# OthmanB/TAMCMC-C-

Measured on AMD Instinct MI355X. Metric: MALA steps/sec (all chains) + achieved HBM GB/s, 64 chains × 1e5-bin spectrum, higher is better.
Workload: dtype f64; 1 GPU; C2: model_MS_Global_a1etaa3_HarveyLike (id 2), 21 modes l=0..2, 56 params, 100000 bins, 64 chains per GPU, trunc_c=20, logL + gradient over 44 variables, params resident in HBM; chains_total=64

## Files before the change

### tamcmc-c-_amd/csrc/tamcmc_dev.h

```cpp
#pragma once
#include <stddef.h>
#include <stdint.h>
#if defined(__HIPCC__)
#define TM_HD __host__ __device__
#else
#define TM_HD
#endif

#define TM_MAXM 7
#define TM_MAXH 3
#define TM_THREADS 256
#define TM_MAXMULT 256
#define TM_GSLOTS 24
#define TM_NSLOTS 16
#define TM_PDEG 8
#define TM_ORDER_MAX 1024
#define TM_HSER 10

#define TM_FAM_GAUSS  0
#define TM_FAM_GLOBAL 1
#define TM_FAM_LOCAL  2

struct TmLayout {
    int32_t model_case;
    int32_t family;
    int32_t variant;
    int32_t Nmax, lmax;
    int32_t Nfl[4];
    int32_t Nsplit, Nwidth, Nnoise, Ninc;
    int32_t off_f[4];
    int32_t s, w, z, q;
    int32_t Nparams;
    int32_t n_mult;
    int32_t nharvey;
    int32_t likelihood_case;
    int32_t Nx;
    int32_t bg_exact;
    int32_t asym_var;
    int32_t pad_l;
    double  x0, xlast, step;
    double  like_p;
};

struct TmMult {
    double g2;
    double aA, aB, c2;
    double nu2[TM_MAXM];
    double hq[TM_MAXM];
    int32_t imin, imax;
    int32_t ncomp;
    int32_t has_asym;
};
static_assert(sizeof(TmMult) == 160, "TmMult layout");
#define TM_MULT_DOUBLES 20

struct TmNoise {
    double H[TM_MAXH];
    double lt[TM_MAXH];
    double p[TM_MAXH];
    double N0;
    double gA, gnu0, gs2;
    int32_t nh;
    int32_t has_gauss;
    int32_t status;
    int32_t pad;
};

static_assert(sizeof(TmNoise) == 120, "TmNoise layout");
#define TM_NOISE_DOUBLES 15

#define TM_UNIT_BINS 512
#define TM_UNIT_SHIFT 9
#define TM_CELL_UNITS 8
#define TM_CELL_SHIFT 3
#ifndef TM_TILE_MAXU
#define TM_TILE_MAXU 8
#endif
#define TM_TILE_MAXU_L 16
#define TM_EQ_MAXU 4096

struct TmCellRec {
    double bg[TM_PDEG + 1];
    double t0[TM_MAXH];
    double lxc;
    int32_t npoly;
    int32_t pad;
};
static_assert(sizeof(TmCellRec) == 8 * (TM_PDEG + 1 + TM_MAXH + 2), "TmCellRec layout");

struct TmTileHdr {
    int32_t u0, u1, nact, cost;
};
static_assert(sizeof(TmTileHdr) == 16, "TmTileHdr layout");

struct TmActive {
    int32_t idx;
    int32_t imin, imax;
    int32_t shape;
};
static_assert(sizeof(TmActive) == 16, "TmActive layout");

struct TmCostModel {
    int32_t c0, a, b, pad;
    int32_t t1, su1, su2, pad2;
};
static inline TM_HD int tm_tile_first_unit(const TmCostModel &g, int su, int t) { return (g.t1 <= 0) ? t * su : (t < g.t1 ? t * g.su1 : g.t1 * g.su1 + (t - g.t1) * g.su2); }
static inline TM_HD int tm_tile_units(const TmCostModel &g, int su, int t) { return (g.t1 <= 0) ? su : (t < g.t1 ? g.su1 : g.su2); }
static inline TM_HD int tm_tile_of_unit(const TmCostModel &g, int su, int u) { return (g.t1 <= 0) ? u / su : (u < g.t1 * g.su1 ? u / g.su1 : g.t1 + (u - g.t1 * g.su1) / g.su2); }

struct TmEvalArgs {
    const double *x2, *y, *lx, *isig2;
    const TmMult *mult;
    const TmNoise *noise;
    const TmCellRec *cell;
    const TmTileHdr *thdr;
    const TmActive *tidx;
    const int32_t *spec;
    const double *wt;
    double *part;
    double *gmult;
    double *gnoise;
    int32_t *ticket;
    double *logL;
    int32_t *status;
    const int32_t *row_of_chain;
    double *model_out;
    int32_t Nx, n_mult, tiles, cells, likelihood_case;
    const int32_t *order;
    int32_t order_mode;
    int32_t prio;
    int32_t generic;
    double like_p;
    unsigned long long tile_magic;
};

static inline int tm_units(long long Nx) { return (int)((Nx + TM_UNIT_BINS - 1) / TM_UNIT_BINS); }
static inline int tm_cells(int units) { return (units + TM_CELL_UNITS - 1) / TM_CELL_UNITS; }
static inline int tm_tiles(int units, int grad)
{
    (void)grad;
    if (units <= 4) return 1;
    if (units < 70) { const int s = units / 10 > 0 ? units / 10 : 1; return (units + s - 1) / s; }
    return (units + TM_TILE_MAXU - 1) / TM_TILE_MAXU;
}

#if defined(__HIPCC__)
#define TM_LN2 0.693147180559945309417232
static __device__ __forceinline__ double tm_tile_logsum(double mant, double e) { return __builtin_fma(e, TM_LN2, log(mant)); }
#endif
static inline TM_HD int tm_setup_balances(int units, int tiles, int equal_cost, int max_units_per_tile)
{
    return (equal_cost != 0 && max_units_per_tile == TM_TILE_MAXU && tiles > 1 && tiles <= TM_ORDER_MAX && units <= TM_EQ_MAXU &&
            (long long)tiles * TM_TILE_MAXU > units) ? 1 : 0;
}

static inline TM_HD int tm_tile_bound(int t, int tiles, int units, const int *pre, long long C, long long cmin)
{
    const long long T = tiles, U = units, S = TM_TILE_MAXU;
    const long long D = T * S - U;
    const long long Nl = (C - T * S * cmin > 0) ? C - T * S * cmin : 0;
    const long long rhs = (long long)t * (D * C + Nl * U);
    int lo = 0, hi = units;
    while (lo < hi) {
        const int mid = (lo + hi) >> 1;
        const long long q = (mid == 0) ? 0 : (long long)pre[mid - 1];
        if (T * (D * q + Nl * mid) >= rhs) hi = mid; else lo = mid + 1;
    }
    return lo;
}

struct TmFusedArgs {
    const double *params, *Tcoefs;
    void *chain_rec, *aux;
    double *hser;
    int32_t p_doubles, pad;
};

#ifdef __cplusplus
extern "C++" {
struct ihipStream_t;
int tm_launch_setup(const TmLayout &L, int Nchains, const double *d_params, const double *d_Tcoefs, double *d_wt, const double *d_lx,
                    int units, int cells, int tiles, int equal_cost, TmCostModel cm, TmMult *d_mult, TmNoise *d_noise, TmCellRec *d_cell,
                    TmTileHdr *d_thdr, TmActive *d_tidx, void *d_chain_rec , void *d_aux ,
                    double *d_hser , int32_t *d_order , void *stream);
size_t tm_sizeof_chain_rec();
size_t tm_sizeof_aux();
int tm_launch_eval(const TmEvalArgs &a, int Nchains, bool grad, void *stream);
int tm_launch_fused(const TmLayout &L, const TmFusedArgs &f, const TmEvalArgs &a, int Nchains, bool grad, void *stream);
int tm_launch_backward(const TmLayout &L, int Nchains, int units, int cells, int tiles, int equal_cost ,
                       TmCostModel geom ,
                       const double *d_params,
                       const double *d_Tcoefs, const void *d_chain_rec, const void *d_aux, const TmNoise *d_noise,
                       const double *d_part, const double *d_gmult, const double *d_gnoise, const TmCellRec *d_cell,
                       const TmTileHdr *d_thdr, const double *d_hser, int Nvars, const int32_t *d_index_to_relax, double *d_grad,
                       double *d_logL, int32_t *d_status, void *stream);
int tm_backward_fits(const TmLayout &L, int tiles, int Nvars);
}
#endif
```

### tamcmc-c-_amd/csrc/tamcmc_eval_body.h

```cpp
#ifndef TAMCMC_EVAL_BODY_H
#define TAMCMC_EVAL_BODY_H
#include <hip/hip_runtime.h>
#include "tamcmc_dev.h"

#define TM_WAVES (TM_THREADS / 64)

typedef const __attribute__((address_space(4))) TmMult *TmMultK;
typedef const __attribute__((address_space(4))) TmCellRec *TmCellRecK;
typedef const __attribute__((address_space(4))) TmTileHdr *TmTileHdrK;
typedef const __attribute__((address_space(4))) TmNoise *TmNoiseK;
typedef const __attribute__((address_space(4))) int32_t *TmIdxK;
typedef const __attribute__((address_space(4))) TmActive *TmActiveK;

typedef int TmEntry __attribute__((ext_vector_type(4)));
__device__ __forceinline__ TmEntry tm_load_entry(TmActiveK p)
{
    return *reinterpret_cast<const __attribute__((address_space(4))) TmEntry *>(p);
}

__device__ __forceinline__ double tm_rcp(double x)
{
    double r = __builtin_amdgcn_rcp(x);
    double e = __builtin_fma(-x, r, 1.0);
    r = __builtin_fma(r, e, r);
    e = __builtin_fma(-x, r, 1.0);
    r = __builtin_fma(r, e, r);
    return r;
}

__device__ __forceinline__ double tm_rcp1(double x)
{
    double r = __builtin_amdgcn_rcp(x);
    const double e = __builtin_fma(-x, r, 1.0);
    return __builtin_fma(r, e, r);
}

template <int MASK>
__device__ __forceinline__ unsigned tm_xor_dw(unsigned v, int lane)
{
    if constexpr (MASK == 1) return __builtin_amdgcn_update_dpp(0u, v, 0xB1, 0xf, 0xf, false);
    else if constexpr (MASK == 2) return __builtin_amdgcn_update_dpp(0u, v, 0x4E, 0xf, 0xf, false);
    else if constexpr (MASK == 4) {
        const unsigned r = __builtin_amdgcn_update_dpp(0u, v, 0x104, 0xf, 0x5, false);
        return __builtin_amdgcn_update_dpp(r, v, 0x114, 0xf, 0xa, false);
    } else if constexpr (MASK == 8) return __builtin_amdgcn_update_dpp(0u, v, 0x128, 0xf, 0xf, false);
    else if constexpr (MASK == 16) {
        const auto r = __builtin_amdgcn_permlane16_swap(v, v, false, false);
        return (lane & 16) ? r[0] : r[1];
    } else {
        const auto r = __builtin_amdgcn_permlane32_swap(v, v, false, false);
        return (lane & 32) ? r[0] : r[1];
    }
}

template <int MASK>
__device__ __forceinline__ double tm_xor(double v, int lane)
{
    const unsigned long long b = __double_as_longlong(v);
    const unsigned lo = tm_xor_dw<MASK>((unsigned)b, lane), hi = tm_xor_dw<MASK>((unsigned)(b >> 32), lane);
    return __longlong_as_double(((unsigned long long)hi << 32) | lo);
}

template <int MASK>
__device__ __forceinline__ double tm_swap_add(double a, double b)
{
    static_assert(MASK == 16 || MASK == 32, "two-register swaps exist for 16 and 32 lanes");
    const unsigned long long ba = __double_as_longlong(a), bb = __double_as_longlong(b);
    unsigned r0l, r1l, r0h, r1h;
    if constexpr (MASK == 32) {
        const auto l = __builtin_amdgcn_permlane32_swap((unsigned)ba, (unsigned)bb, false, false);
        const auto h = __builtin_amdgcn_permlane32_swap((unsigned)(ba >> 32), (unsigned)(bb >> 32), false, false);
        r0l = l[0]; r1l = l[1]; r0h = h[0]; r1h = h[1];
    } else {
        const auto l = __builtin_amdgcn_permlane16_swap((unsigned)ba, (unsigned)bb, false, false);
        const auto h = __builtin_amdgcn_permlane16_swap((unsigned)(ba >> 32), (unsigned)(bb >> 32), false, false);
        r0l = l[0]; r1l = l[1]; r0h = h[0]; r1h = h[1];
    }
    const double r0 = __longlong_as_double(((unsigned long long)r0h << 32) | r0l);
    const double r1 = __longlong_as_double(((unsigned long long)r1h << 32) | r1l);
    return r0 + r1;
}

__device__ __forceinline__ double tm_wave_sum(double v)
{
    const int lane = threadIdx.x & 63;
    v += tm_xor<32>(v, lane);
    v += tm_xor<16>(v, lane);
    v += tm_xor<8>(v, lane);
    v += tm_xor<4>(v, lane);
    v += tm_xor<2>(v, lane);
    v += tm_xor<1>(v, lane);
    return v;
}

__device__ __forceinline__ double tm_wave_prod(double v)
{
    const int lane = threadIdx.x & 63;
    v *= tm_xor<32>(v, lane);
    v *= tm_xor<16>(v, lane);
    v *= tm_xor<8>(v, lane);
    v *= tm_xor<4>(v, lane);
    v *= tm_xor<2>(v, lane);
    v *= tm_xor<1>(v, lane);
    return v;
}


__device__ __forceinline__ double tm_poly(TmCellRecK tr, double z)
{
    double p = tr->bg[TM_PDEG];
#pragma unroll
    for (int j = TM_PDEG - 1; j >= 0; j--) p = __builtin_fma(p, z, tr->bg[j]);
    return p;
}

template <int N, int MASK>
struct TmBfly {
    static constexpr int NE = (N + 1) & ~1;
    static constexpr int H = NE / 2;
    __device__ static __forceinline__ void run(double (&v)[TM_GSLOTS], int lane)
    {
        if constexpr (N == 1) {
            v[0] += tm_xor<MASK>(v[0], lane);
        } else if constexpr (MASK >= 16) {
#pragma unroll
            for (int i = 0; i < H; i++) v[i] = tm_swap_add<MASK>(v[i], (i + H < N) ? v[i + H] : 0.0);
        } else {
            const bool hi = (lane & MASK) != 0;
#pragma unroll
            for (int i = 0; i < H; i++) {
                const double up = (i + H < N) ? v[i + H] : 0.0;
                const double send = hi ? v[i] : up;
                const double keep = hi ? up : v[i];
                v[i] = keep + tm_xor<MASK>(send, lane);
            }
        }
        if constexpr (MASK > 1) TmBfly<(N == 1 ? 1 : H), MASK / 2>::run(v, lane);
    }
    __device__ static __forceinline__ int slot_of(int lane, bool &valid)
    {
        if constexpr (N == 1) {
            return 0;
        } else {
            int sub = 0;
            if constexpr (MASK > 1) sub = TmBfly<H, MASK / 2>::slot_of(lane, valid);
            const int idx = sub + (((lane & MASK) != 0) ? H : 0);
            if (idx >= N) valid = false;
            return idx;
        }
    }
};

template <int NC>
__device__ __forceinline__ double tm_mult_value(double x2, const double (&nu2)[NC], const double (&hq)[NC], double g2,
                                                double (&d)[NC], double (&r)[NC])
{
    double E[NC], P[NC];
#pragma unroll
    for (int m = 0; m < NC; m++) {
        d[m] = x2 - nu2[m];
        E[m] = __builtin_fma(d[m], d[m], g2);
    }
    P[0] = E[0];
#pragma unroll
    for (int m = 1; m < NC; m++) P[m] = P[m - 1] * E[m];
    double inv = tm_rcp1(P[NC - 1]);
    double s = 0.0;
#pragma unroll
    for (int m = NC - 1; m >= 1; m--) {
        r[m] = inv * P[m - 1];
        inv = inv * E[m];
    }
    r[0] = inv;
#pragma unroll
    for (int m = 0; m < NC; m++) s = __builtin_fma(hq[m], r[m], s);
    return s;
}

template <int NC>
__device__ __forceinline__ double tm_mult_sum(double x2, const double (&nu2)[NC], const double (&hq)[NC], double g2)
{
    double d = x2 - nu2[0];
    double Q = __builtin_fma(d, d, g2);
    double N = hq[0];
#pragma unroll
    for (int m = 1; m < NC; m++) {
        d = x2 - nu2[m];
        const double E = __builtin_fma(d, d, g2);
        N = __builtin_fma(hq[m], Q, N * E);
        Q = Q * E;
    }
    return N * tm_rcp(Q);
}

template <int NC, int KG, bool ASYM>
__device__ __forceinline__ void tm_accum_mult(TmMultK sm, const double (&x2)[KG], const int (&bi)[KG], double (&acc)[KG], const bool edge)
{
    double nu2[NC], hq[NC];
#pragma unroll
    for (int m = 0; m < NC; m++) { nu2[m] = sm->nu2[m]; hq[m] = sm->hq[m]; }
    const double g2 = sm->g2;
    const double aAh = ASYM ? 0.5 * sm->aA : 0.0, aB = ASYM ? sm->aB : 1.0, c2 = ASYM ? sm->c2 : 0.0;
    double s[KG];
#pragma unroll
    for (int k = 0; k < KG; k++) {
        s[k] = tm_mult_sum<NC>(x2[k], nu2, hq, g2);
        if (ASYM) {
            const double a = __builtin_fma(x2[k], aAh, aB);
            s[k] = s[k] * __builtin_fma(a, a, c2);
        }
    }
    if (edge) {
        const int imin = sm->imin, imax = sm->imax;
#pragma unroll
        for (int k = 0; k < KG; k++) {
            const bool inside = (bi[k] >= imin) && (bi[k] < imax);
            s[k] = inside ? s[k] : 0.0;
        }
    }
#pragma unroll
    for (int k = 0; k < KG; k++) acc[k] += s[k];
}

template <int KG>
__device__ __forceinline__ void tm_accum_dispatch(TmMultK sm, const int shape, const double (&x2)[KG], const int (&bi)[KG], double (&acc)[KG], const bool edge)
{
    switch (shape) {
    case 1: tm_accum_mult<1, KG, false>(sm, x2, bi, acc, edge); break;
    case 3: tm_accum_mult<3, KG, false>(sm, x2, bi, acc, edge); break;
    case 5: tm_accum_mult<5, KG, false>(sm, x2, bi, acc, edge); break;
    case 7: tm_accum_mult<7, KG, false>(sm, x2, bi, acc, edge); break;
    case 256 + 1: tm_accum_mult<1, KG, true>(sm, x2, bi, acc, edge); break;
    case 256 + 3: tm_accum_mult<3, KG, true>(sm, x2, bi, acc, edge); break;
    case 256 + 5: tm_accum_mult<5, KG, true>(sm, x2, bi, acc, edge); break;
    default: tm_accum_mult<7, KG, true>(sm, x2, bi, acc, edge); break;
    }
}

template <int NC> struct TmGradSlots {
    static constexpr int L = (NC - 1) / 2;
    static constexpr int A0 = NC, C = NC + L + 1, ASYM0 = NC + L + 2;
    __device__ static constexpr int count(bool asym) { return asym ? ASYM0 + 3 : ASYM0; }
};
template <int NC> __device__ __forceinline__ int tm_grad_store_slot(int v)
{
    using SL = TmGradSlots<NC>;
    return (v < NC) ? v : (v < SL::C) ? 7 + (v - NC) : (v == SL::C) ? 11 : 21 + (v - SL::ASYM0);
}

template <int NC, bool ASYM>
__device__ __forceinline__ void tm_grad_unit(const double (&nu2)[NC], const double (&hq)[NC], double g2, double aAh, double aB, double c2,
                                             int imin, int imax, const double *__restrict__ gx, const double *wq, int i0, int Nx,
                                             const bool edge, double (&g)[TM_GSLOTS])
{
    using SL = TmGradSlots<NC>;
#pragma unroll
    for (int k = 0; k < 2; k++) {
        double x2, wk;
        if (edge) {
            const int i = i0 + k * TM_THREADS;
            const bool inside = (i >= imin) && (i < imax) && (i < Nx);
            x2 = gx[i < Nx ? i : Nx - 1];
            wk = inside ? wq[k * TM_THREADS] : 0.0;
        } else {
            x2 = gx[i0 + k * TM_THREADS];
            wk = wq[k * TM_THREADS];
        }
        double d[NC], r[NC];
        const double Sv = tm_mult_value<NC>(x2, nu2, hq, g2, d, r);
        double wA = wk;
        if (ASYM) {
            const double a = __builtin_fma(x2, aAh, aB);
            wA = wk * __builtin_fma(a, a, c2);
            const double ws = wk * Sv;
            g[SL::ASYM0 + 0] += ws;
            g[SL::ASYM0 + 1] = __builtin_fma(ws, a, g[SL::ASYM0 + 1]);
            g[SL::ASYM0 + 2] = __builtin_fma(ws * a, 0.5 * x2, g[SL::ASYM0 + 2]);
        }
#pragma unroll
        for (int m = 0; m < NC; m++) {
            const double t1 = wA * r[m];
            const double t2 = t1 * r[m];
            const int am = (m >= SL::L) ? m - SL::L : SL::L - m;
            g[SL::A0 + am] += t1;
            g[m] = __builtin_fma(t2, d[m], g[m]);
            g[SL::C] = __builtin_fma(hq[m], t2, g[SL::C]);
        }
    }
}

template <int NC, bool ASYM>
__device__ __forceinline__ void tm_grad_mult(TmMultK sm, const double *__restrict__ gx, const double *s_w,
                                             int u0, int u1, int Nx, int tid, int lane, double *s_red_row)
{
    constexpr int V = TmGradSlots<NC>::count(ASYM);
    double g[TM_GSLOTS];
    double nu2[NC], hq[NC];
#pragma unroll
    for (int m = 0; m < NC; m++) { nu2[m] = sm->nu2[m]; hq[m] = sm->hq[m]; }
    const double g2 = sm->g2;
    const int imin = sm->imin, imax = sm->imax;
    const double aAh = ASYM ? 0.5 * sm->aA : 0.0, aB = ASYM ? sm->aB : 1.0, c2 = ASYM ? sm->c2 : 0.0;
#pragma unroll
    for (int s = 0; s < TM_GSLOTS; s++) g[s] = 0.0;
#pragma unroll 1
    for (int u = u0; u < u1; u++) {
        const int lo = u << TM_UNIT_SHIFT, hi = lo + TM_UNIT_BINS;
        if (hi <= imin || lo >= imax) continue;
        const double *wq = s_w + (u - u0) * TM_UNIT_BINS + tid;
        tm_grad_unit<NC, ASYM>(nu2, hq, g2, aAh, aB, c2, imin, imax, gx, wq, lo + tid, Nx, !(lo >= imin && hi <= imax && hi <= Nx), g);
    }
#if defined(TM_ABLATE) && (TM_ABLATE & 1)
    if (lane == 0) s_red_row[0] = g[0] + g[1] + g[2];
    return;
#endif
    TmBfly<V, 32>::run(g, lane);
    constexpr int NSPLIT = (V > 16) ? 5 : (V > 8) ? 4 : (V > 4) ? 3 : (V > 2) ? 2 : 1;
    const int lowmask = (64 >> NSPLIT) - 1;
    bool valid = true;
    const int slot = TmBfly<V, 32>::slot_of(lane, valid);
    if ((lane & lowmask) == 0 && valid) {
        s_red_row[tm_grad_store_slot<NC>(slot)] = g[0];
    }
}

#ifndef TM_LB_FWD
#define TM_LB_FWD 4
#endif
#ifndef TM_LB_GRAD
#define TM_LB_GRAD 4
#endif
#ifdef TM_TRACE
__device__ unsigned long long *g_tm_trace = nullptr;
#define TM_STAMP(slot) do { if (threadIdx.x == 0 && g_tm_trace) g_tm_trace[((size_t)blockIdx.y * gridDim.x + blockIdx.x) * 4 + (slot)] = wall_clock64(); } while (0)
#else
#define TM_STAMP(slot) do { } while (0)
#endif

template <int N> struct TmInt { static constexpr int value = N; };
template <bool B> struct TmBool { static constexpr bool value = B; };

template <bool GRAD, bool GEN = true>
__device__ __forceinline__ void tm_eval_body(const TmEvalArgs &a, const int chain, const int tile, double *s_w)
{
    const int like = GEN ? a.likelihood_case : 0;
    const int tid = threadIdx.x;
    const int lane = tid & 63, wave = tid >> 6;
    TmNoiseK sn = (TmNoiseK)(a.noise + chain);

#if defined(TM_ABLATE) && (TM_ABLATE & 16)
    if (a.Nx > 0) return;
#endif
    __shared__ double s_red[2][TM_WAVES][TM_GSLOTS];

    const size_t spec_off = (a.spec != nullptr) ? (size_t)((TmIdxK)a.spec)[chain] * (size_t)a.Nx : 0;
    const double *__restrict__ yp = a.y + spec_off;
    const double *__restrict__ isp = a.isig2 + spec_off;
    const TmMult *__restrict__ gm = a.mult + (size_t)chain * a.n_mult;
    TmTileHdrK th = (TmTileHdrK)(a.thdr + (size_t)chain * a.tiles + tile);
    const int u0 = th->u0;
    int u1 = th->u1;
    if (u1 - u0 > (GRAD ? TM_TILE_MAXU : TM_TILE_MAXU_L)) u1 = u0 + (GRAD ? TM_TILE_MAXU : TM_TILE_MAXU_L);
    const int nact = th->nact;
    TmCellRecK cells = (TmCellRecK)(a.cell + (size_t)chain * a.cells);
    TmActiveK tix = (TmActiveK)(a.tidx + ((size_t)chain * a.tiles + tile) * (a.n_mult > 0 ? a.n_mult : 1));
    const int nh = sn->nh;
    const bool has_gauss = GEN && sn->has_gauss != 0;
    const double N0 = sn->N0;
    const int row = (GEN && a.row_of_chain != nullptr) ? a.row_of_chain[chain] : -1;
    const double *__restrict__ xb = a.x2;
    const double *__restrict__ lb = a.lx;

#if defined(TM_ABLATE) && (TM_ABLATE & 32)
    if (nact >= 0 && N0 == N0) { if (tid == 0 && !GRAD) a.part[((size_t)chain * a.tiles + tile) * 4] = (double)(nh + row + u0 + (has_gauss ? 1 : 0)); return; }
#endif
    double S1 = 0.0;
    double P = 1.0;
    int esum = 0;
    int sgn = 0;
    double gn_[GRAD ? TM_GSLOTS : 1];
#pragma unroll
    for (int s_ = 0; s_ < (GRAD ? TM_GSLOTS : 1); s_++) gn_[s_] = 0.0;
    const double wscale = GRAD ? a.wt[2 * chain + 1] : 0.0;

    auto group = [&](auto kg_c, auto full_c, const int u, TmCellRecK tr) __attribute__((always_inline)) {
        constexpr int KG = decltype(kg_c)::value;
        constexpr bool FULL = decltype(full_c)::value;
        const int lo = u << TM_UNIT_SHIFT, hi = lo + KG * TM_THREADS;
        double x2[KG], acc[KG];
        int bi[KG];
#pragma unroll
        for (int k = 0; k < KG; k++) {
            const int i = lo + k * TM_THREADS + tid;
            if (FULL) {
                bi[k] = i;
                x2[k] = xb[(unsigned)i];
            } else {
                const bool valid = i < a.Nx;
                bi[k] = valid ? i : -1;
                x2[k] = a.x2[valid ? i : a.Nx - 1];
            }
            acc[k] = 0.0;
        }
        constexpr bool EARLY = FULL && !GRAD;
        double lxe[EARLY ? KG : 1], ye[EARLY ? KG : 1];
        if constexpr (EARLY) {
#pragma unroll
            for (int k = 0; k < KG; k++) { lxe[k] = (nh > 0) ? lb[(unsigned)bi[k]] : 0.0; ye[k] = yp[(unsigned)bi[k]]; }
        }
        if constexpr (GRAD) {
            for (int jj = 0; jj < nact; jj++) {
                const int idx = tix[jj].idx, imin = tix[jj].imin, imax = tix[jj].imax, shape = tix[jj].shape;
                if (hi <= imin || lo >= imax) continue;
                tm_accum_dispatch<KG>((TmMultK)(gm + idx), shape, x2, bi, acc, !(FULL && lo >= imin && hi <= imax));
            }
        } else if (nact > 0) {
            TmEntry e = tm_load_entry(tix);
            asm volatile("" :: "s"(e.x));
            for (int jj = 0; jj < nact; jj++) {
                const TmEntry en = tm_load_entry(tix + (jj + 1 < nact ? jj + 1 : jj));
                const int idx = e.x, imin = e.y, imax = e.z, shape = e.w;
                if (!(hi <= imin || lo >= imax))
                    tm_accum_dispatch<KG>((TmMultK)(gm + idx), shape, x2, bi, acc, !(FULL && lo >= imin && hi <= imax));
                e = en;
            }
        }

        constexpr int KH = GRAD ? 2 : KG;
        const bool npoly = tr->npoly != 0;
#pragma unroll
        for (int h0 = 0; h0 < KG; h0 += KH) {
        double hu[TM_MAXH][GRAD ? KH : 1], harg[GRAD ? KH : 1];
        bool n0_done = false;
        if (nh > 0) {
            double dl[KH];
#pragma unroll
            for (int k = 0; k < KH; k++) {
#if defined(TM_ABLATE) && (TM_ABLATE & 128)
                dl[k] = tr->lxc + 1e-9 * x2[h0 + k];
#else
                dl[k] = EARLY ? lxe[h0 + k] : FULL ? lb[(unsigned)bi[h0 + k]] : a.lx[bi[h0 + k] >= 0 ? bi[h0 + k] : a.Nx - 1];
#endif
                if constexpr (GRAD) harg[k] = dl[k];
            }
            if (npoly) {
                const double lxc = tr->lxc;
#pragma unroll
                for (int k = 0; k < KH; k++) { dl[k] -= lxc; acc[h0 + k] += tm_poly(tr, dl[k]); if constexpr (GRAD) harg[k] = dl[k]; }
                n0_done = true;
            } else {
#pragma unroll
                for (int h = 0; h < TM_MAXH; h++) {
                    if (h < nh) {
                        const double Hh = sn->H[h], ph = sn->p[h], lth = sn->lt[h];
#pragma unroll
                        for (int k = 0; k < KH; k++) {
                            const double t = exp(ph * (lth + dl[k]));
                            const double uu = 1.0 / (t + 1.0);
                            acc[h0 + k] += Hh * uu;
                            if constexpr (GRAD) hu[h][k] = uu;
                        }
                    }
                }
            }
        }
        if (has_gauss) {
            const double gA = sn->gA, gnu0 = sn->gnu0, gs2 = sn->gs2;
#pragma unroll
            for (int k = 0; k < KH; k++) {
                const double dd = 0.5 * x2[h0 + k] - gnu0;
                acc[h0 + k] = gA * exp((-0.5 * (dd * dd)) / gs2) + acc[h0 + k];
            }
        }
        if (!n0_done) {
#pragma unroll
            for (int k = 0; k < KH; k++) acc[h0 + k] += N0;
        }
        if (row >= 0) {
#pragma unroll
            for (int k = 0; k < KH; k++)
                if (FULL || bi[h0 + k] >= 0) a.model_out[(size_t)row * a.Nx + (size_t)(lo + (h0 + k) * TM_THREADS + tid)] = acc[h0 + k];
        }

        double wreg[GRAD ? KH : 1];
        if (like == 0) {
#pragma unroll
            for (int k = 0; k < KH; k++) {
                double wv = 0.0;
                if (FULL || bi[h0 + k] >= 0) {
                    const double M = acc[h0 + k];
                    const double yv = EARLY ? ye[h0 + k] : FULL ? yp[(unsigned)bi[h0 + k]] : yp[bi[h0 + k]];
                    sgn |= __double2hiint(M);
                    const double rM = tm_rcp(M);
                    S1 = __builtin_fma(yv, rM, S1);
                    int e;
                    P *= frexp(M, &e);
                    esum += e;
                    wv = wscale * (yv * rM * rM - rM);
                }
                if constexpr (GRAD) wreg[k] = wv;
            }
            {
                int e;
                P = frexp(P, &e);
                esum += e;
            }
        } else {
#pragma unroll
            for (int k = 0; k < KH; k++) {
                double wv = 0.0;
                if (FULL || bi[h0 + k] >= 0) {
                    const int i = lo + (h0 + k) * TM_THREADS + tid;
                    const double dd = yp[i] - acc[h0 + k];
                    const double is2 = isp[i];
                    S1 = __builtin_fma(dd * dd, is2, S1);
                    wv = wscale * dd * is2;
                }
                if constexpr (GRAD) wreg[k] = wv;
            }
        }
        if constexpr (GRAD) {
#pragma unroll
            for (int k = 0; k < KH; k++) {
                const double wk = wreg[k];
                s_w[((u - u0) * 2 + h0 + k) * TM_THREADS + tid] = wk;
                gn_[3 * TM_MAXH] += wk;
#if defined(TM_ABLATE) && (TM_ABLATE & 512)
                if (false) {
#else
                if (nh > 0 && npoly) {
#endif
                    double q = wk;
#pragma unroll
                    for (int j = 0; j < TM_HSER - 1; j++) { q *= harg[k]; gn_[j] += q; }
                } else if (nh > 0) {
#pragma unroll
                    for (int h = 0; h < TM_MAXH; h++) {
                        if (h < nh) {
                            const double wu = wk * hu[h][k];
                            const double tu2 = wu * (1.0 - hu[h][k]);
                            gn_[3 * h] += wu;
                            gn_[3 * h + 1] += tu2;
                            gn_[3 * h + 2] = __builtin_fma(tu2, sn->lt[h] + harg[k], gn_[3 * h + 2]);
                        }
                    }
                }
                if (has_gauss) {
                    const double dd = 0.5 * x2[h0 + k] - sn->gnu0;
                    const double we = wk * exp((-0.5 * (dd * dd)) / sn->gs2);
                    gn_[13] += we;
                    gn_[14] = __builtin_fma(we, dd, gn_[14]);
                    gn_[15] = __builtin_fma(we * dd, dd, gn_[15]);
                }
            }
        }
        if constexpr (GRAD) __builtin_amdgcn_sched_barrier(0);
        }
    };

    auto flush_noise = [&](const int part) __attribute__((always_inline)) {
        if constexpr (GRAD) {
            static_assert(TM_NSLOTS == 16, "butterfly below assumes 16 noise slots");
            TmBfly<TM_NSLOTS, 32>::run(gn_, lane);
            bool valid = true;
            const int slot = TmBfly<TM_NSLOTS, 32>::slot_of(lane, valid);
            double *red = s_red[1][wave];
            if ((lane & 3) == 0) red[slot] = gn_[0];
            __syncthreads();
            if (tid < TM_NSLOTS) {
                double t = 0.0;
#pragma unroll
                for (int wv = 0; wv < TM_WAVES; wv++) t += s_red[1][wv][tid];
                a.gnoise[(((size_t)chain * a.tiles + tile) * 2 + part) * TM_NSLOTS + tid] = t;
            }
            __syncthreads();
#pragma unroll
            for (int s_ = 0; s_ < TM_GSLOTS; s_++) gn_[s_] = 0.0;
        }
    };

    {
        const int cell0 = u0 >> TM_CELL_SHIFT;
        int cur_cell = cell0;
        auto cell_of = [&](const int uu) __attribute__((always_inline)) {
            const int ce = uu >> TM_CELL_SHIFT;
            if (GRAD && ce != cur_cell) { flush_noise(0); cur_cell = ce; }
            return cells + ce;
        };
        int u = u0;
#if defined(TM_ABLATE) && (TM_ABLATE & 256)
        u = u1;
#endif
        if ((u & 1) && u < u1 && ((u + 1) << TM_UNIT_SHIFT) <= a.Nx) { TmCellRecK tr = cell_of(u); group(TmInt<2>(), TmBool<true>(), u, tr); u += 1; }
#pragma unroll 1
        for (; u + 2 <= u1 && ((u + 2) << TM_UNIT_SHIFT) <= a.Nx; u += 2) { TmCellRecK tr = cell_of(u); group(TmInt<4>(), TmBool<true>(), u, tr); }
#pragma unroll 1
        for (; u < u1; u += 1) {
            TmCellRecK tr = cell_of(u);
            if (((u + 1) << TM_UNIT_SHIFT) <= a.Nx) group(TmInt<2>(), TmBool<true>(), u, tr);
            else                                    group(TmInt<2>(), TmBool<false>(), u, tr);
        }
        if (GRAD) flush_noise(cur_cell - cell0);
    }
    TM_STAMP(1);
    double Pm = 1.0, Pe = 0.0;
    if (like == 0) {
        int e;
        Pm = frexp(tm_wave_prod(P), &e);
        Pe = tm_wave_sum((double)esum) + (double)e;
        if (__builtin_amdgcn_ballot_w64(sgn < 0) != 0) Pm = __builtin_nan("");
    }
    S1 = tm_wave_sum(S1);
    if (lane == 0) { s_red[0][wave][0] = S1; s_red[0][wave][1] = Pm; s_red[0][wave][2] = Pe; }
    __syncthreads();
    if constexpr (GRAD) {
        if (tid == 0) {
            double t1 = 0.0, tm = 1.0, te = 0.0;
#pragma unroll
            for (int wv = 0; wv < TM_WAVES; wv++) { t1 += s_red[0][wv][0]; tm *= s_red[0][wv][1]; te += s_red[0][wv][2]; }
            double *out = a.part + ((size_t)chain * a.tiles + tile) * 4;
            out[0] = t1;
            out[1] = tm;
            out[2] = te;
        }
    } else if (wave == 0) {
        int last = 0;
        double *pp = a.part + (size_t)chain * a.tiles * 4;
        if (lane == 0) {
            double t1 = 0.0, tm = 1.0, te = 0.0;
#pragma unroll
            for (int wv = 0; wv < TM_WAVES; wv++) { t1 += s_red[0][wv][0]; tm *= s_red[0][wv][1]; te += s_red[0][wv][2]; }
#if defined(TM_ABLATE) && (TM_ABLATE & 4)
            pp[4 * tile] = t1; pp[4 * tile + 1] = tm; pp[4 * tile + 2] = te;
#else
            if (a.tiles == 1) {
                pp[0] = t1; pp[1] = tm; pp[2] = te;
                const double t2 = (like == 0) ? tm_tile_logsum(tm, te) : 0.0;
                double f = (like == 0) ? -a.like_p * (t1 + t2) : -t1;
                f = f / a.wt[2 * chain];
                int st = a.noise[chain].status;
                if (st != 0) f = __builtin_nan("");
                else if (!(f == f)) st = 1;
                a.logL[chain] = f;
                if (a.status) a.status[chain] = st;
            } else {
            __hip_atomic_store(pp + 4 * tile, t1, __ATOMIC_RELAXED, __HIP_MEMORY_SCOPE_AGENT);
            __hip_atomic_store(pp + 4 * tile + 1, tm, __ATOMIC_RELAXED, __HIP_MEMORY_SCOPE_AGENT);
            __hip_atomic_store(pp + 4 * tile + 2, te, __ATOMIC_RELAXED, __HIP_MEMORY_SCOPE_AGENT);
            asm volatile("s_waitcnt vmcnt(0)" ::: "memory");
            const int prev = __hip_atomic_fetch_add(a.ticket + chain, 1, __ATOMIC_RELAXED, __HIP_MEMORY_SCOPE_AGENT);
            last = (prev == a.tiles - 1) ? 1 : 0;
            }
#endif
        }
        last = __shfl(last, 0, 64);
        if (last) {
            double s1 = 0.0, s2 = 0.0;
            for (int t = lane; t < a.tiles; t += 64) {
                s1 += __hip_atomic_load(pp + 4 * t, __ATOMIC_RELAXED, __HIP_MEMORY_SCOPE_AGENT);
                if (like == 0)
                    s2 += tm_tile_logsum(__hip_atomic_load(pp + 4 * t + 1, __ATOMIC_RELAXED, __HIP_MEMORY_SCOPE_AGENT),
                                         __hip_atomic_load(pp + 4 * t + 2, __ATOMIC_RELAXED, __HIP_MEMORY_SCOPE_AGENT));
            }
            s1 = tm_wave_sum(s1);
            s2 = tm_wave_sum(s2);
            if (lane == 0) {
                double f = (like == 0) ? -a.like_p * (s1 + s2) : -s1;
                f = f / a.wt[2 * chain];
                int st = a.noise[chain].status;
                if (st != 0) f = __builtin_nan("");
                else if (!(f == f)) st = 1;
                a.logL[chain] = f;
                if (a.status) a.status[chain] = st;
                __hip_atomic_store(a.ticket + chain, 0, __ATOMIC_RELAXED, __HIP_MEMORY_SCOPE_AGENT);
            }
        }
    }

    TM_STAMP(2);
#ifdef TM_TRACE
    if (threadIdx.x == 0 && g_tm_trace) {
        unsigned hw;
        asm volatile("s_getreg_b32 %0, hwreg(HW_REG_HW_ID)" : "=s"(hw));
        unsigned xcc;
        asm volatile("s_getreg_b32 %0, hwreg(HW_REG_XCC_ID)" : "=s"(xcc));
        g_tm_trace[((size_t)blockIdx.y * gridDim.x + blockIdx.x) * 4 + 3] = ((unsigned long long)xcc << 32) | hw;
    }
#endif
    if constexpr (GRAD) {
        __syncthreads();
#if defined(TM_ABLATE) && (TM_ABLATE & 2)
        for (int jj = 0; jj < 0; jj++) {
#else
        for (int jj = 0; jj < nact; jj++) {
#endif
            const int idx = tix[jj].idx, shape = tix[jj].shape;
            TmMultK sm = (TmMultK)(gm + idx);
            const int nc = shape & 255;
            double *red = s_red[(jj + 1) & 1][wave];
            if (lane == 0) {
                const int Lm = (nc - 1) >> 1;
                for (int am = Lm + 1; am <= 3; am++) red[7 + am] = 0.0;
                if (shape < 256) { red[21] = 0.0; red[22] = 0.0; red[23] = 0.0; }
            }
            switch (shape) {
            case 1: tm_grad_mult<1, false>(sm, a.x2, s_w, u0, u1, a.Nx, tid, lane, red); break;
            case 3: tm_grad_mult<3, false>(sm, a.x2, s_w, u0, u1, a.Nx, tid, lane, red); break;
            case 5: tm_grad_mult<5, false>(sm, a.x2, s_w, u0, u1, a.Nx, tid, lane, red); break;
            case 7: tm_grad_mult<7, false>(sm, a.x2, s_w, u0, u1, a.Nx, tid, lane, red); break;
            case 256 + 1: tm_grad_mult<1, true>(sm, a.x2, s_w, u0, u1, a.Nx, tid, lane, red); break;
            case 256 + 3: tm_grad_mult<3, true>(sm, a.x2, s_w, u0, u1, a.Nx, tid, lane, red); break;
            case 256 + 5: tm_grad_mult<5, true>(sm, a.x2, s_w, u0, u1, a.Nx, tid, lane, red); break;
            default: tm_grad_mult<7, true>(sm, a.x2, s_w, u0, u1, a.Nx, tid, lane, red); break;
            }
#if defined(TM_ABLATE) && (TM_ABLATE & 64)
            if (tid < TM_GSLOTS) a.gmult[(((size_t)chain * a.tiles + tile) * a.n_mult + idx) * TM_GSLOTS + tid] = red[tid];
#else
            __syncthreads();
            if (tid < TM_GSLOTS) {
                double t = 0.0;
                if (tid < nc || (tid >= 7 && tid < 12) || tid >= 21) {
#pragma unroll
                    for (int wv = 0; wv < TM_WAVES; wv++) t += s_red[(jj + 1) & 1][wv][tid];
                }
                a.gmult[(((size_t)chain * a.tiles + tile) * a.n_mult + idx) * TM_GSLOTS + tid] = t;
            }
#endif
        }
        TM_STAMP(2);
    }
}

#endif
```

Baseline: 680,600 chain-steps/s (model+logL+grad).

## Accumulate Lorentzian sum as a single rational fraction to avoid per-mode reciprocals

The forward model sum over Lorentzian profiles is kept as a running numerator/denominator pair (N/Q) per bin. Each new profile is merged by cross-multiplication, and only one reciprocal is taken at the end instead of one per mode. This removes the many reciprocal/division operations in the hot accumulation loop. In exchange it adds extra multiplies, periodic frexp/ldexp renormalisation every few components to avoid overflow, and a small accuracy risk. The y preload is also deferred to save registers.

```diff
diff --git a/tamcmc-c-_amd/csrc/tamcmc_dev.h b/tamcmc-c-_amd/csrc/tamcmc_dev.h
--- a/tamcmc-c-_amd/csrc/tamcmc_dev.h
+++ b/tamcmc-c-_amd/csrc/tamcmc_dev.h
@@ -169,6 +169,30 @@
     return lo;
 }
 
+#define TM_RAT_K 12
+static inline TM_HD void tm_rat_step(double &N, double &Q, double h, double E)
+{
+    N = __builtin_fma(h, Q, N * E);
+    Q = Q * E;
+}
+static inline TM_HD void tm_rat_merge(double &N, double &Q, double Nk, double Qk)
+{
+    N = __builtin_fma(Nk, Q, N * Qk);
+    Q = Q * Qk;
+}
+static inline TM_HD void tm_rat_renorm(double &N, double &Q)
+{
+    int e;
+    Q = __builtin_frexp(Q, &e);
+    N = __builtin_ldexp(N, -e);
+}
+static inline TM_HD int tm_rat_count(int &nf, int nc)
+{
+    const int r = (nf + nc > TM_RAT_K) ? 1 : 0;
+    nf = r ? nc : nf + nc;
+    return r;
+}
+
 struct TmFusedArgs {
     const double *params, *Tcoefs;
     void *chain_rec, *aux;
diff --git a/tamcmc-c-_amd/csrc/tamcmc_eval_body.h b/tamcmc-c-_amd/csrc/tamcmc_eval_body.h
--- a/tamcmc-c-_amd/csrc/tamcmc_eval_body.h
+++ b/tamcmc-c-_amd/csrc/tamcmc_eval_body.h
@@ -220,6 +220,68 @@
     }
 #pragma unroll
     for (int k = 0; k < KG; k++) acc[k] += s[k];
+}
+
+#ifndef TM_MERGE
+#define TM_MERGE 1
+#endif
+
+template <int NC, int KG, bool ASYM, bool SPLIT>
+__device__ __forceinline__ void tm_merge_mult(TmMultK sm, const double (&x2)[KG], const int (&bi)[KG], double (&N)[KG], double (&Q)[KG], const bool edge)
+{
+    double nu2[NC], hq[NC];
+#pragma unroll
+    for (int m = 0; m < NC; m++) { nu2[m] = sm->nu2[m]; hq[m] = sm->hq[m]; }
+    const double g2 = sm->g2;
+    const double aAh = ASYM ? 0.5 * sm->aA : 0.0, aB = ASYM ? sm->aB : 1.0, c2 = ASYM ? sm->c2 : 0.0;
+    constexpr int KS = (SPLIT && KG > 2) ? 2 : KG;
+    static_assert(KG % KS == 0, "bins are taken KS at a time");
+#pragma unroll
+    for (int k0 = 0; k0 < KG; k0 += KS) {
+        double Nk[KS], Qk[KS];
+#pragma unroll
+        for (int k = 0; k < KS; k++) {
+            double d = x2[k0 + k] - nu2[0];
+            Qk[k] = __builtin_fma(d, d, g2);
+            Nk[k] = hq[0];
+#pragma unroll
+            for (int m = 1; m < NC; m++) {
+                d = x2[k0 + k] - nu2[m];
+                tm_rat_step(Nk[k], Qk[k], hq[m], __builtin_fma(d, d, g2));
+            }
+            if (ASYM) {
+                const double a = __builtin_fma(x2[k0 + k], aAh, aB);
+                Nk[k] = Nk[k] * __builtin_fma(a, a, c2);
+            }
+        }
+        if (edge) {
+            const int imin = sm->imin, imax = sm->imax;
+#pragma unroll
+            for (int k = 0; k < KS; k++) {
+                const bool inside = (bi[k0 + k] >= imin) && (bi[k0 + k] < imax);
+                Nk[k] = inside ? Nk[k] : 0.0;
+                Qk[k] = inside ? Qk[k] : 1.0;
+            }
+        }
+#pragma unroll
+        for (int k = 0; k < KS; k++) tm_rat_merge(N[k0 + k], Q[k0 + k], Nk[k], Qk[k]);
+        if constexpr (KS < KG) __builtin_amdgcn_sched_barrier(0);
+    }
+}
+
+template <int KG, bool SPLIT>
+__device__ __forceinline__ void tm_merge_dispatch(TmMultK sm, const int shape, const double (&x2)[KG], const int (&bi)[KG], double (&N)[KG], double (&Q)[KG], const bool edge)
+{
+    switch (shape) {
+    case 1: tm_merge_mult<1, KG, false, SPLIT>(sm, x2, bi, N, Q, edge); break;
+    case 3: tm_merge_mult<3, KG, false, SPLIT>(sm, x2, bi, N, Q, edge); break;
+    case 5: tm_merge_mult<5, KG, false, SPLIT>(sm, x2, bi, N, Q, edge); break;
+    case 7: tm_merge_mult<7, KG, false, SPLIT>(sm, x2, bi, N, Q, edge); break;
+    case 256 + 1: tm_merge_mult<1, KG, true, SPLIT>(sm, x2, bi, N, Q, edge); break;
+    case 256 + 3: tm_merge_mult<3, KG, true, SPLIT>(sm, x2, bi, N, Q, edge); break;
+    case 256 + 5: tm_merge_mult<5, KG, true, SPLIT>(sm, x2, bi, N, Q, edge); break;
+    default: tm_merge_mult<7, KG, true, SPLIT>(sm, x2, bi, N, Q, edge); break;
+    }
 }
 
 template <int KG>
@@ -403,12 +465,31 @@
             acc[k] = 0.0;
         }
         constexpr bool EARLY = FULL && !GRAD;
-        double lxe[EARLY ? KG : 1], ye[EARLY ? KG : 1];
+        constexpr bool EARLY_Y = EARLY && !TM_MERGE;
+        double lxe[EARLY ? KG : 1], ye[EARLY_Y ? KG : 1];
         if constexpr (EARLY) {
 #pragma unroll
-            for (int k = 0; k < KG; k++) { lxe[k] = (nh > 0) ? lb[(unsigned)bi[k]] : 0.0; ye[k] = yp[(unsigned)bi[k]]; }
-        }
-        if constexpr (GRAD) {
+            for (int k = 0; k < KG; k++) { lxe[k] = (nh > 0) ? lb[(unsigned)bi[k]] : 0.0; if constexpr (EARLY_Y) ye[k] = yp[(unsigned)bi[k]]; }
+        }
+        if constexpr (GRAD && TM_MERGE) {
+            double rn[KG], rq[KG];
+#pragma unroll
+            for (int k = 0; k < KG; k++) { rn[k] = 0.0; rq[k] = 1.0; }
+            int nf = 0;
+            for (int jj = 0; jj < nact; jj++) {
+                const int idx = tix[jj].idx, imin = tix[jj].imin, imax = tix[jj].imax, shape = tix[jj].shape;
+                if (hi <= imin || lo >= imax) continue;
+                if (tm_rat_count(nf, shape & 255)) {
+#pragma unroll
+                    for (int k = 0; k < KG; k++) tm_rat_renorm(rn[k], rq[k]);
+                }
+                tm_merge_dispatch<KG, !GRAD>((TmMultK)(gm + idx), shape, x2, bi, rn, rq, !(FULL && lo >= imin && hi <= imax));
+            }
+            if (nf > 0) {
+#pragma unroll
+                for (int k = 0; k < KG; k++) acc[k] = rn[k] * tm_rcp(rq[k]);
+            }
+        } else if constexpr (GRAD) {
             for (int jj = 0; jj < nact; jj++) {
                 const int idx = tix[jj].idx, imin = tix[jj].imin, imax = tix[jj].imax, shape = tix[jj].shape;
                 if (hi <= imin || lo >= imax) continue;
@@ -417,13 +498,34 @@
         } else if (nact > 0) {
             TmEntry e = tm_load_entry(tix);
             asm volatile("" :: "s"(e.x));
+#if TM_MERGE
+            double rn[KG], rq[KG];
+#pragma unroll
+            for (int k = 0; k < KG; k++) { rn[k] = 0.0; rq[k] = 1.0; }
+            int nf = 0;
+#endif
             for (int jj = 0; jj < nact; jj++) {
                 const TmEntry en = tm_load_entry(tix + (jj + 1 < nact ? jj + 1 : jj));
                 const int idx = e.x, imin = e.y, imax = e.z, shape = e.w;
-                if (!(hi <= imin || lo >= imax))
+                if (!(hi <= imin || lo >= imax)) {
+#if TM_MERGE
+                    if (tm_rat_count(nf, shape & 255)) {
+#pragma unroll
+                        for (int k = 0; k < KG; k++) tm_rat_renorm(rn[k], rq[k]);
+                    }
+                    tm_merge_dispatch<KG, !GRAD>((TmMultK)(gm + idx), shape, x2, bi, rn, rq, !(FULL && lo >= imin && hi <= imax));
+#else
                     tm_accum_dispatch<KG>((TmMultK)(gm + idx), shape, x2, bi, acc, !(FULL && lo >= imin && hi <= imax));
+#endif
+                }
                 e = en;
             }
+#if TM_MERGE
+            if (nf > 0) {
+#pragma unroll
+                for (int k = 0; k < KG; k++) acc[k] = rn[k] * tm_rcp(rq[k]);
+            }
+#endif
         }
 
         constexpr int KH = GRAD ? 2 : KG;
@@ -489,7 +591,7 @@
                 double wv = 0.0;
                 if (FULL || bi[h0 + k] >= 0) {
                     const double M = acc[h0 + k];
-                    const double yv = EARLY ? ye[h0 + k] : FULL ? yp[(unsigned)bi[h0 + k]] : yp[bi[h0 + k]];
+                    const double yv = EARLY_Y ? ye[h0 + k] : FULL ? yp[(unsigned)bi[h0 + k]] : yp[bi[h0 + k]];
                     sgn |= __double2hiint(M);
                     const double rM = tm_rcp(M);
                     S1 = __builtin_fma(yv, rM, S1);
```

After: 687,200 chain-steps/s (model+logL+grad), median of 6. No clear change (+1.0%).
